# YonkaMayonkaZ/NCF

Hardware: NVIDIA B200
Metric: NeuMF train samples/s (higher is better)
Workload: dtype f32

## Files before the change

### ncf_b200/csrc/tile_umma.cu

```cuda
#include <algorithm>
#include <cstdlib>

#include "common.cuh"
#include "tile_params.cuh"

namespace {

constexpr int kTile = 128;
constexpr uint32_t kHiMask = 0xffffe000u;
constexpr int kProducerWarps = 8;
constexpr int kLoaderWarp = 17;
constexpr int kGemmThreads = 576;
constexpr int kMaxStages = 4;

enum { EPI_RELU_STORE = 0, EPI_PREDICT = 1, EPI_PREDICT_TRAIN = 2, EPI_MASK_STORE = 3, EPI_SCATTER = 4 };

struct GemmArgs {
  int K;
  int N;
  int n_total;
  int passes;
  int layer;
  int gather;
  int stages;
  int ablate;
  const float* a;
  const float* b_img;
  const float* bias;
  float* out;
  const float* mask_src;
};

struct WgradJob {
  int k, mb, nb, cta0, nctas;
  int S;
};
struct WgradArgs {
  int njobs, passes, ablate;
  WgradJob job[12];
};

__device__ __forceinline__ uint32_t smem_u32(const void* p) { return (uint32_t)__cvta_generic_to_shared(p); }

__device__ __forceinline__ void mbar_init(uint64_t* b, uint32_t count) {
  asm volatile("mbarrier.init.shared::cta.b64 [%0], %1;" ::"r"(smem_u32(b)), "r"(count));
}
__device__ __forceinline__ void mbar_arrive(uint64_t* b) {
  asm volatile("mbarrier.arrive.shared::cta.b64 _, [%0];" ::"r"(smem_u32(b)) : "memory");
}
__device__ __forceinline__ void mbar_expect_tx(uint64_t* b, uint32_t bytes) {
  asm volatile("mbarrier.arrive.expect_tx.shared::cta.b64 _, [%0], %1;" ::"r"(smem_u32(b)), "r"(bytes) : "memory");
}
__device__ __forceinline__ void mbar_wait(uint64_t* b, uint32_t parity) {
  const uint32_t addr = smem_u32(b);
  for (uint32_t spin = 0; spin < (1u << 26); ++spin) {
    uint32_t done;
#ifdef NCF_MBAR_POLL
    asm volatile(
        "{\n\t.reg .pred p;\n\tmbarrier.test_wait.parity.shared::cta.b64 p, [%1], %2;\n\tselp.u32 %0, 1, 0, p;\n\t}"
        : "=r"(done) : "r"(addr), "r"(parity) : "memory");
#else
    asm volatile(
        "{\n\t.reg .pred p;\n\tmbarrier.try_wait.parity.shared::cta.b64 p, [%1], %2;\n\tselp.u32 %0, 1, 0, p;\n\t}"
        : "=r"(done) : "r"(addr), "r"(parity) : "memory");
#endif
    if (done) return;
  }
  __trap();
}
__device__ __forceinline__ bool mbar_test_warp(uint64_t* b, uint32_t parity) {
  uint32_t done = 0;
  if ((threadIdx.x & 31) == 0)
    asm volatile(
        "{\n\t.reg .pred p;\n\tmbarrier.test_wait.parity.shared::cta.b64 p, [%1], %2;\n\tselp.u32 %0, 1, 0, p;\n\t}"
        : "=r"(done) : "r"(smem_u32(b)), "r"(parity) : "memory");
  return __shfl_sync(0xffffffffu, done, 0) != 0;
}
__device__ __forceinline__ void mbar_wait_warp(uint64_t* b, uint32_t parity) {
  if ((threadIdx.x & 31) == 0) mbar_wait(b, parity);
  __syncwarp();
}
__device__ __forceinline__ void mbar_arrive_warp(uint64_t* b) {
  __syncwarp();
  if ((threadIdx.x & 31) == 0) mbar_arrive(b);
}
__device__ __forceinline__ void bulk_g2s(void* dst, const void* src, uint32_t bytes, uint64_t* bar) {
  asm volatile("cp.async.bulk.shared::cluster.global.mbarrier::complete_tx::bytes [%0], [%1], %2, [%3];"
               ::"r"(smem_u32(dst)), "l"(src), "r"(bytes), "r"(smem_u32(bar)) : "memory");
}
__device__ __forceinline__ void cp_async16_zfill(void* dst, const void* src, bool valid) {
  asm volatile("cp.async.cg.shared.global [%0], [%1], 16, %2;" ::"r"(smem_u32(dst)), "l"(src), "r"(valid ? 16 : 0) : "memory");
}
__device__ __forceinline__ void fence_async_smem() { asm volatile("fence.proxy.async.shared::cta;" ::: "memory"); }
__device__ __forceinline__ void tc_fence_before() { asm volatile("tcgen05.fence::before_thread_sync;" ::: "memory"); }
__device__ __forceinline__ void tc_fence_after() { asm volatile("tcgen05.fence::after_thread_sync;" ::: "memory"); }
__device__ __forceinline__ void tc_commit(uint64_t* bar) {
  asm volatile("tcgen05.commit.cta_group::1.mbarrier::arrive::one.shared::cluster.b64 [%0];" ::"r"(smem_u32(bar)) : "memory");
}
__device__ __forceinline__ void tc_mma(uint32_t d_tmem, uint64_t da, uint64_t db, uint32_t idesc, uint32_t accumulate) {
  asm volatile(
      "{\n\t.reg .pred p;\n\tsetp.ne.b32 p, %4, 0;\n\t"
      "tcgen05.mma.cta_group::1.kind::tf32 [%0], %1, %2, %3, p;\n\t}"
      ::"r"(d_tmem), "l"(da), "l"(db), "r"(idesc), "r"(accumulate) : "memory");
}
__device__ __forceinline__ void tc_ld32(uint32_t taddr, float (&v)[32]) {
  uint32_t r[32];
  asm volatile(
      "tcgen05.ld.sync.aligned.32x32b.x32.b32 "
      "{%0,%1,%2,%3,%4,%5,%6,%7,%8,%9,%10,%11,%12,%13,%14,%15,"
      "%16,%17,%18,%19,%20,%21,%22,%23,%24,%25,%26,%27,%28,%29,%30,%31}, [%32];"
      : "=r"(r[0]), "=r"(r[1]), "=r"(r[2]), "=r"(r[3]), "=r"(r[4]), "=r"(r[5]), "=r"(r[6]), "=r"(r[7]),
        "=r"(r[8]), "=r"(r[9]), "=r"(r[10]), "=r"(r[11]), "=r"(r[12]), "=r"(r[13]), "=r"(r[14]), "=r"(r[15]),
        "=r"(r[16]), "=r"(r[17]), "=r"(r[18]), "=r"(r[19]), "=r"(r[20]), "=r"(r[21]), "=r"(r[22]), "=r"(r[23]),
        "=r"(r[24]), "=r"(r[25]), "=r"(r[26]), "=r"(r[27]), "=r"(r[28]), "=r"(r[29]), "=r"(r[30]), "=r"(r[31])
      : "r"(taddr));
  asm volatile("tcgen05.wait::ld.sync.aligned;" ::: "memory");
#pragma unroll
  for (int j = 0; j < 32; ++j) v[j] = __uint_as_float(r[j]);
// ... 15 lines not shown
  d |= (uint32_t)a_mn << 15;
  d |= (uint32_t)b_mn << 16;
  d |= (uint32_t)(n >> 3) << 17;
  d |= (uint32_t)(m >> 4) << 24;
  return d;
}

__device__ __forceinline__ void split4(const float4 x, float4& hi, float4& lo) {
  hi.x = __uint_as_float(__float_as_uint(x.x) & kHiMask);
  hi.y = __uint_as_float(__float_as_uint(x.y) & kHiMask);
  hi.z = __uint_as_float(__float_as_uint(x.z) & kHiMask);
  hi.w = __uint_as_float(__float_as_uint(x.w) & kHiMask);
  lo = make_float4(x.x - hi.x, x.y - hi.y, x.z - hi.z, x.w - hi.w);
}

__device__ __forceinline__ float warp_colsum32(float (&v)[32], int lane) {
#pragma unroll
  for (int o = 16; o > 0; o >>= 1) {
    const bool upper = (lane & o) != 0;
#pragma unroll
    for (int i = 0; i < o; ++i) {
      const float send = upper ? v[i] : v[i + o];
      const float keep = upper ? v[i + o] : v[i];
      v[i] = keep + __shfl_xor_sync(0xffffffffu, send, o);
    }
  }
  return v[0];
}

__device__ __forceinline__ void named_bar(int id, int count) {
  asm volatile("bar.sync %0, %1;" ::"r"(id), "r"(count) : "memory");
}

__global__ void umma_weight_images_kernel(const TileParams p) {
  const int k = blockIdx.y >> 1, dir = blockIdx.y & 1;
  const int kin = p.W[k], nout = p.W[k + 1];
  const int rows = dir ? kin : nout, K = dir ? nout : kin;
  const int panels = (K + 31) / 32;
  const float* w = p.w[k];
  float* img = dir ? p.wsplit_b[k] : p.wsplit_f[k];
  const int64_t total = (int64_t)panels * rows * 32;
  for (int64_t idx = blockIdx.x * (int64_t)blockDim.x + threadIdx.x; idx < total;
       idx += (int64_t)gridDim.x * blockDim.x) {
    const int cc = (int)(idx & 31);
    const int r = (int)((idx >> 5) % rows);
    const int pi = (int)((idx >> 5) / rows);
    const int c = pi * 32 + cc;
    float x = 0.f;
    if (c < K) x = dir ? w[(int64_t)c * kin + r] : w[(int64_t)r * kin + c];
    const float hi = __uint_as_float(__float_as_uint(x) & kHiMask);
    const int64_t off = (int64_t)pi * 2 * rows * 32 + (int64_t)r * 32 + ((((cc >> 2) ^ (r & 7)) << 2) | (cc & 3));
    img[off] = hi;
    img[off + (int64_t)rows * 32] = x - hi;
  }
}

#ifdef NCF_UMMA_TRACE
__device__ long long g_trace[3][128];
#define NCF_TRACE(role, slot) do { if (blockIdx.x == 0 && blockIdx.y == 0 && (slot) < 128) g_trace[role][slot] = clock64(); } while (0)
#else
#define NCF_TRACE(role, slot) do { } while (0)
#endif

struct GemmBars {
  uint64_t full[kMaxStages], empty[kMaxStages], acc_full[2], acc_empty[2];
  uint32_t tmem_base;
  float pg[2 * 128 + 4];
// ... 358 lines not shown
          }
        }
      }
      tc_fence_before();
      if (q == 0 && lane == 0) NCF_TRACE(2, 2 * (int)lt + 1);
      mbar_arrive_warp(&bars.acc_empty[a]);
    }
  }
  tc_fence_before();
  __syncthreads();
  if (EPI == EPI_PREDICT_TRAIN)
    for (int i = tid; i <= p.predict_size; i += kGemmThreads) atomicAdd(&p.gt[p.pw_off + i], bars.pg[i]);
  if (warp == kProducerWarps) asm volatile("tcgen05.dealloc.cta_group::1.sync.aligned.b32 %0, %1;" ::"r"(tmem), "r"(tmem_cols));
}

constexpr int kMaxGemms = 2 * NCF_MAX_LAYERS;
constexpr int kRingMax = 6;
constexpr int kBStages = 3;

struct TowerGemm {
  int kind;
  int k, N, K;
  int a_hi, a_lo;
  int d_col;
  int n_total, row0;
  int new_operand;
  const float* img;
};
struct TowerArgs {
  int passes, ng, ablate;
  int ring_col, ring_stages;
  int hcol[NCF_MAX_LAYERS + 1], lcol[NCF_MAX_LAYERS + 1];
  TowerGemm gemm[kMaxGemms];
};

struct TowerBars {
  uint64_t a_full[kRingMax], a_empty[kRingMax], b_full[kBStages], b_empty[kBStages];
  uint64_t acc_ready[2], opnd_ready, tile_done, dl_ready;
  uint64_t panel_ready[8];
  uint32_t tmem_base;
  float pg[2 * 64 + 8];
  float xch[kTile];
};

__device__ __forceinline__ void tc_st32(uint32_t taddr, const float (&v)[32]) {
  asm volatile(
      "tcgen05.st.sync.aligned.32x32b.x32.b32 [%0], {%1,%2,%3,%4,%5,%6,%7,%8,%9,%10,%11,%12,%13,%14,%15,%16,"
      "%17,%18,%19,%20,%21,%22,%23,%24,%25,%26,%27,%28,%29,%30,%31,%32};"
      ::"r"(taddr), "r"(__float_as_uint(v[0])), "r"(__float_as_uint(v[1])), "r"(__float_as_uint(v[2])),
        "r"(__float_as_uint(v[3])), "r"(__float_as_uint(v[4])), "r"(__float_as_uint(v[5])), "r"(__float_as_uint(v[6])),
        "r"(__float_as_uint(v[7])), "r"(__float_as_uint(v[8])), "r"(__float_as_uint(v[9])), "r"(__float_as_uint(v[10])),
        "r"(__float_as_uint(v[11])), "r"(__float_as_uint(v[12])), "r"(__float_as_uint(v[13])), "r"(__float_as_uint(v[14])),
        "r"(__float_as_uint(v[15])), "r"(__float_as_uint(v[16])), "r"(__float_as_uint(v[17])), "r"(__float_as_uint(v[18])),
        "r"(__float_as_uint(v[19])), "r"(__float_as_uint(v[20])), "r"(__float_as_uint(v[21])), "r"(__float_as_uint(v[22])),
        "r"(__float_as_uint(v[23])), "r"(__float_as_uint(v[24])), "r"(__float_as_uint(v[25])), "r"(__float_as_uint(v[26])),
        "r"(__float_as_uint(v[27])), "r"(__float_as_uint(v[28])), "r"(__float_as_uint(v[29])), "r"(__float_as_uint(v[30])),
        "r"(__float_as_uint(v[31])) : "memory");
}
__device__ __forceinline__ void tc_wait_st() { asm volatile("tcgen05.wait::st.sync.aligned;" ::: "memory"); }
__device__ __forceinline__ void tc_mma_ts(uint32_t d_tmem, uint32_t a_tmem, uint64_t db, uint32_t idesc, uint32_t accumulate) {
  asm volatile(
      "{\n\t.reg .pred p;\n\tsetp.ne.b32 p, %4, 0;\n\t"
      "tcgen05.mma.cta_group::1.kind::tf32 [%0], [%1], %2, %3, p;\n\t}"
      ::"r"(d_tmem), "r"(a_tmem), "l"(db), "r"(idesc), "r"(accumulate) : "memory");
}
__device__ __forceinline__ float lo_of(float x) { return x - __uint_as_float(__float_as_uint(x) & kHiMask); }
// ... 36 lines not shown
  extern __shared__ __align__(1024) uint8_t smem_raw[];
  __shared__ TowerBars bars;
  uint8_t* smem = reinterpret_cast<uint8_t*>((reinterpret_cast<uintptr_t>(smem_raw) + 1023) & ~(uintptr_t)1023);
  const int tid = threadIdx.x, warp = tid >> 5, lane = tid & 31;
  const int L = p.L;
  const int64_t ntiles = (p.B + kTile - 1) / kTile;
  const int64_t my_tiles = (blockIdx.x < ntiles) ? (ntiles - blockIdx.x + gridDim.x - 1) / gridDim.x : 0;
  const int P0 = p.W[0] >> 5;
  const uint32_t b_stage = 128u * 256u;
  uint8_t* land = smem + kBStages * b_stage;
  const int NA = g.ring_stages;

  if (tid == 0) {
    const int nm = (g.passes == 3) ? 3 : 1;
    for (int s = 0; s < NA; ++s) { mbar_init(&bars.a_full[s], 4); mbar_init(&bars.a_empty[s], nm); }
    for (int s = 0; s < kBStages; ++s) { mbar_init(&bars.b_full[s], 1); mbar_init(&bars.b_empty[s], nm); }
    mbar_init(&bars.acc_ready[0], nm * kTowerMmaSets);
    mbar_init(&bars.acc_ready[1], nm * kTowerMmaSets);
    mbar_init(&bars.opnd_ready, kTowerEpiWarps);
    for (int c = 0; c < 8; ++c) mbar_init(&bars.panel_ready[c], 4);
    mbar_init(&bars.tile_done, kTowerEpiWarps);
    mbar_init(&bars.dl_ready, kTowerEpiWarps / 2);
    asm volatile("fence.mbarrier_init.release.cluster;" ::: "memory");
  }
  for (int i = tid; i < 2 * 64 + 8; i += kTowerThreads) bars.pg[i] = 0.f;
  if (warp == 8) {
    asm volatile("tcgen05.alloc.cta_group::1.sync.aligned.shared::cta.b32 [%0], 512;" ::"r"(smem_u32(&bars.tmem_base)));
    asm volatile("tcgen05.relinquish_alloc_permit.cta_group::1.sync.aligned;");
  }
  tc_fence_before();
  __syncthreads();
  tc_fence_after();
  const uint32_t tmem = bars.tmem_base;

  if (warp < 8) {
    const int grp = warp >> 2, q = warp & 3;
    const int r = q * 32 + lane;
    const int d = p.d;
    const int own = P0 / 2;
    const uint32_t lane_addr = tmem + ((uint32_t)(q * 32) << 16);
    int s = grp;
    uint32_t ph = 0;
    auto copy_panel = [&](int64_t tl, int pi, int64_t uu, int64_t ii) {
      const bool ok = tl < my_tiles && uu >= 0 && uu < p.U && ii >= 0 && ii < p.I && !(g.ablate & 1);
      const int c0 = pi * 32;
      const float* src = p.eum;
      if (ok) src = (c0 < d) ? p.eum + uu * d + c0 : p.eim + ii * d + (c0 - d);
      uint8_t* dst = land + pi * (kTile * 128) + r * 128;
#pragma unroll
      for (int c = 0; c < 8; ++c) cp_async16_zfill(dst + ((c ^ (r & 7)) << 4), src + c * 4, ok);
      asm volatile("cp.async.commit_group;" ::: "memory");
    };
    auto row_idx = [&](int64_t tl, int64_t& uu, int64_t& ii) {
      uu = -1;
      ii = -1;
      const int64_t row = (blockIdx.x + tl * gridDim.x) * kTile + r;
      if (tl < my_tiles && row < p.B) {
        uu = p.user[p.user_div > 0 ? row / p.user_div : row];
        ii = p.item[row];
      }
    };
    int64_t nu, nit;
    row_idx(0, nu, nit);
    for (int j = 0; j < own; ++j) copy_panel(0, grp + 2 * j, nu, nit);
    const int f = p.f;
    const bool has_gmf = p.type != NCF_MLP;
// ... 338 lines not shown
#pragma unroll
            for (int j = 0; j < 32; ++j) v[j] = (x[j] > 0.f) ? v[j] : 0.f;
            tc_st32(lane_addr + g.lcol[k] + c0, v);
            if (g.passes == 3) {
#pragma unroll
              for (int j = 0; j < 32; ++j) x[j] = lo_of(v[j]);
              tc_st32(lane_addr + g.hcol[k] + c0, x);
            }
            quad8_transpose(v, lane);
            tc_wait_st();
            tc_fence_before();
            mbar_arrive_warp(&bars.panel_ready[c0 >> 5]);
            store_rows_t(v, p.delta[k], N, row - lane, p.B, c0, lane);
          }
        } else {
          for (int c0 = c_begin; c0 < c_end; c0 += 32) {
            tc_ld32(lane_addr + G.d_col + c0, v);
            quad8_transpose(v, lane);
            const int col = G.row0 + c0;
            const bool to_user = col < dmlp;
            const int64_t my_idx = ok ? (to_user ? u : it) : -1;
            float* tab = (to_user ? p.gum + col : p.gim + (col - dmlp)) + 4 * (lane & 7);
#pragma unroll
            for (int i = 0; i < 8; ++i) {
              const int64_t idx = __shfl_sync(0xffffffffu, my_idx, (lane & ~7) + i);
              if (idx >= 0) red_add4(tab + idx * dmlp, make_float4(v[4 * i], v[4 * i + 1], v[4 * i + 2], v[4 * i + 3]));
            }
          }
        }
        if (zero_late) zero_cols(g.gemm[0].d_col, g.gemm[0].N);
        tc_wait_st();
        tc_fence_before();
        if (warp == kTowerEpiWarp0 + 1 && lane == 0) NCF_TRACE(2, 2 * ((int)tl * g.ng + gi) + 1);
        if (gi + 1 == g.ng) mbar_arrive_warp(&bars.tile_done);
      }
    }
  }
  tc_fence_before();
  __syncthreads();
  if (TRAIN)
    for (int i = tid; i <= p.predict_size; i += kTowerThreads) atomicAdd(&p.gt[p.pw_off + i], bars.pg[i]);
  if (warp == 8) asm volatile("tcgen05.dealloc.cta_group::1.sync.aligned.b32 %0, 512;" ::"r"(tmem));
}

constexpr int kWgProducerWarps = 8;
constexpr int kWgProducers = kWgProducerWarps * 32;
constexpr int kWgradThreads = kWgProducers + 96;

constexpr int kWgStages = 2;
struct WgradBars {
  uint64_t full[kWgStages], empty[kWgStages], acc_full;
  uint32_t tmem_base;
  float db[128];
};

__device__ __forceinline__ uint32_t mn_offset(int s, int fo, int S) {
  const int panel = fo >> 5, cc = fo & 31;
  return (uint32_t)(panel * (S * 128) + s * 128 + (((cc >> 3) ^ (s & 3)) << 5) + ((cc & 7) << 2));
}

__global__ void __launch_bounds__(kWgradThreads, 1)
umma_wgrad_kernel(const __grid_constant__ TileParams p, const __grid_constant__ WgradArgs g) {
  extern __shared__ __align__(1024) uint8_t smem_raw[];
  __shared__ WgradBars bars;
  uint8_t* smem = reinterpret_cast<uint8_t*>((reinterpret_cast<uintptr_t>(smem_raw) + 1023) & ~(uintptr_t)1023);
  const int tid = threadIdx.x, warp = tid >> 5, lane = tid & 31;
  int ji = 0;
  while (ji + 1 < g.njobs && (int)blockIdx.x >= g.job[ji + 1].cta0) ++ji;
  const WgradJob job = g.job[ji];
  const int k = job.k, kin = p.W[k], nout = p.W[k + 1];
  const int MB = min(128, nout - job.mb * 128), NB = min(256, kin - job.nb * 256);
  const int local = (int)blockIdx.x - job.cta0;
  const int S = job.S;
  const int64_t nchunks = (p.B + S - 1) / S;
  const uint32_t a_img = (uint32_t)MB * S * 4, b_img = (uint32_t)NB * S * 4;
  const uint32_t stage_bytes = 2 * a_img + 2 * b_img;
  const int64_t my_chunks = (local < nchunks) ? (nchunks - local + job.nctas - 1) / job.nctas : 0;

  if (tid == 0) {
    const int nm = (g.passes == 3) ? 3 : 1;
    for (int s = 0; s < kWgStages; ++s) { mbar_init(&bars.full[s], kWgProducerWarps); mbar_init(&bars.empty[s], nm); }
    mbar_init(&bars.acc_full, nm);
    asm volatile("fence.mbarrier_init.release.cluster;" ::: "memory");
  }
  if (tid < 128) bars.db[tid] = 0.f;
  if (warp == kWgProducerWarps) {
    asm volatile("tcgen05.alloc.cta_group::1.sync.aligned.shared::cta.b32 [%0], 256;" ::"r"(smem_u32(&bars.tmem_base)));
    asm volatile("tcgen05.relinquish_alloc_permit.cta_group::1.sync.aligned;");
  }
  tc_fence_before();
  __syncthreads();
  tc_fence_after();
  const uint32_t tmem = bars.tmem_base;
  if (warp < kWgProducerWarps) {
    float z[32];
#pragma unroll
    for (int j = 0; j < 32; ++j) z[j] = 0.f;
    for (int c0 = (warp >> 2) * 128; c0 < (warp >> 2) * 128 + 128; c0 += 32)
      tc_st32(tmem + ((uint32_t)((warp & 3) * 32) << 16) + c0, z);
    tc_wait_st();
  }
  tc_fence_before();
  __syncthreads();
  tc_fence_after();

  if (warp < kWgProducerWarps) {
    const int t = tid, d = p.d;
    const float* delta = p.delta[k + 1];
    const float* actk = (k > 0) ? p.act[k] : nullptr;
    const int pa = MB >> 2, pb = NB >> 2;
    const int na = S * pa / kWgProducers, nbp = S * pb / kWgProducers;
    const int ca = t % pa, sa0 = t / pa, sas = kWgProducers / pa;
    const int cb = t % pb, sb0 = t / pb, sbs = kWgProducers / pb;
    float4 dbsum = make_float4(0.f, 0.f, 0.f, 0.f);
    const int fo = job.nb * 256 + cb * 4;
    const bool from_user = fo < d;
    const int64_t* idx_src = from_user ? p.user : p.item;
    const float* tab = from_user ? p.eum + fo : p.eim + (fo - d);
    const int64_t idx_lim = from_user ? p.U : p.I;
    int64_t idx_even[8], idx_odd[8];
    auto issue_idx = [&](int64_t ci, int64_t (&idxv)[8]) {
      const int64_t row0 = (local + ci * job.nctas) * S;
#pragma unroll
      for (int i = 0; i < 8; ++i) {
        const int64_t row = row0 + sb0 + i * sbs;
        idxv[i] = (i < nbp && ci < my_chunks && row < p.B) ? idx_src[row] : -1;
      }
    };
    auto issue = [&](int64_t ci, bool blocking) -> bool {
      const int s = (int)(ci % kWgStages);
      const uint32_t par = (uint32_t)((ci / kWgStages) & 1) ^ 1;
      if (blocking) mbar_wait_warp(&bars.empty[s], par);
      else if (!mbar_test_warp(&bars.empty[s], par)) return false;
      if (t == 0) NCF_TRACE(0, 2 * (int)ci);
      uint8_t* st = smem + (size_t)s * stage_bytes;
      const int64_t row0 = (local + ci * job.nctas) * S;
      const bool off = (g.ablate & 64) != 0;
#pragma unroll
      for (int i = 0; i < 4; ++i) {
        if (i < na) {
          const int64_t row = row0 + sa0 + i * sas;
          const bool ok = row < p.B && !off;
          cp_async16_zfill(st + mn_offset(sa0 + i * sas, ca * 4, S),
                           ok ? delta + row * nout + job.mb * 128 + ca * 4 : delta, ok);
        }
      }
#pragma unroll
      for (int i = 0; i < 8; ++i) {
        if (i < nbp) {
          const float* src;
          bool ok;
          if (k == 0) {
            const int64_t ix = (ci & 1) ? idx_odd[i] : idx_even[i];
            ok = ix >= 0 && ix < idx_lim && !off;
            src = ok ? tab + ix * d : tab;
          } else {
            const int64_t row = row0 + sb0 + i * sbs;
            ok = row < p.B && !off;
            src = ok ? actk + row * kin + fo : actk;
          }
          cp_async16_zfill(st + 2 * a_img + mn_offset(sb0 + i * sbs, cb * 4, S), src, ok);
        }
      }
      asm volatile("cp.async.commit_group;" ::: "memory");
      if (k == 0) {
        if (ci & 1) issue_idx(ci + 2, idx_odd);
        else issue_idx(ci + 2, idx_even);
      }
      return true;
    };
    auto consume = [&](int64_t ci, int newer) {
      const int s = (int)(ci % kWgStages);
      uint8_t* st = smem + (size_t)s * stage_bytes;
      if (newer >= 3) asm volatile("cp.async.wait_group 3;" ::: "memory");
      else if (newer == 2) asm volatile("cp.async.wait_group 2;" ::: "memory");
      else if (newer == 1) asm volatile("cp.async.wait_group 1;" ::: "memory");
      else asm volatile("cp.async.wait_group 0;" ::: "memory");
      if (!(g.ablate & 256)) {
#pragma unroll
        for (int i = 0; i < 4; ++i) {
          if (i < na) {
            const uint32_t off = mn_offset(sa0 + i * sas, ca * 4, S);
            const float4 x = *reinterpret_cast<const float4*>(st + off);
            float4 hi, lo;
            split4(x, hi, lo);
            dbsum.x += x.x; dbsum.y += x.y; dbsum.z += x.z; dbsum.w += x.w;
            if (g.ablate & 512) *reinterpret_cast<float4*>(st + off) = x;
            if (g.passes == 3) *reinterpret_cast<float4*>(st + a_img + off) = lo;
          }
        }
#pragma unroll
        for (int i = 0; i < 8; ++i) {
          if (i < nbp && g.passes == 3) {
            const uint32_t off = 2 * a_img + mn_offset(sb0 + i * sbs, cb * 4, S);
            const float4 x = *reinterpret_cast<const float4*>(st + off);
            float4 hi, lo;
            split4(x, hi, lo);
            if (g.ablate & 512) *reinterpret_cast<float4*>(st + off) = x;
            *reinterpret_cast<float4*>(st + b_img + off) = lo;
          }
        }
      }
      fence_async_smem();
      if (t == 0) NCF_TRACE(0, 2 * (int)ci + 1);
      mbar_arrive_warp(&bars.full[s]);
    };
    if (k == 0) {
      issue_idx(0, idx_even);
      issue_idx(1, idx_odd);
    }
    int64_t issued = 0;
    for (int64_t ci = 0; ci < my_chunks; ++ci) {
      if (issued == ci) issue(issued++, true);
      while (issued < my_chunks && issued - ci < kWgStages && issue(issued, false)) ++issued;
      consume(ci, (int)(issued - ci - 1));
    }
    if (job.nb == 0) {
      atomicAdd(&bars.db[ca * 4 + 0], dbsum.x);
      atomicAdd(&bars.db[ca * 4 + 1], dbsum.y);
      atomicAdd(&bars.db[ca * 4 + 2], dbsum.z);
      atomicAdd(&bars.db[ca * 4 + 3], dbsum.w);
    }
    named_bar(1, kWgProducers);
    if (job.nb == 0 && t < MB && my_chunks > 0) atomicAdd(&p.gt[p.b_off[k] + job.mb * 128 + t], bars.db[t]);
    if (my_chunks > 0) {
      mbar_wait_warp(&bars.acc_full, 0);
      tc_fence_after();
      const int q = warp & 3, part = warp >> 2, parts = min(kWgProducerWarps / 4, NB / 32);
      const int m = q * 32 + lane;
      float* dst = p.gt + p.w_off[k] + (int64_t)(job.mb * 128 + m) * kin + job.nb * 256;
      float v[32];
      for (int c0 = part * (NB / parts); c0 < (part + 1) * (NB / parts) && part < parts; c0 += 32) {
        tc_ld32(tmem + ((uint32_t)(q * 32) << 16) + c0, v);
        if (m < MB && !(g.ablate & 32)) {
#pragma unroll
          for (int j = 0; j < 32; j += 4) red_add4(dst + c0 + j, make_float4(v[j], v[j + 1], v[j + 2], v[j + 3]));
        }
      }
    }
  } else if (lane == 0 && (warp == kWgProducerWarps || g.passes == 3)) {
    const int pass = warp - kWgProducerWarps;
    const uint32_t idesc = make_idesc(128, NB, 1, 1);
    for (int64_t ci = 0; ci < my_chunks; ++ci) {
      const int s = (int)(ci % kWgStages);
      mbar_wait(&bars.full[s], (uint32_t)(ci / kWgStages) & 1);
      if (pass == 0) NCF_TRACE(1, 2 * (int)ci);
      tc_fence_after();
      const uint32_t base = smem_u32(smem + (size_t)s * stage_bytes);
      const uint32_t ahi = base, alo = base + a_img, bhi = base + 2 * a_img, blo = bhi + b_img;
      const uint64_t da0 = make_desc(pass == 1 ? alo : ahi, S * 128, 512, 1);
      const uint64_t db0 = make_desc(pass == 2 ? blo : bhi, S * 128, 512, 1);
      for (int ks = 0; ks < ((g.ablate & 128) ? 0 : S / 8); ++ks) tc_mma(tmem, da0 + 64 * ks, db0 + 64 * ks, idesc, 1u);
      tc_commit(&bars.empty[s]);
      if (pass == 0) NCF_TRACE(1, 2 * (int)ci + 1);
    }
    if (my_chunks > 0) tc_commit(&bars.acc_full);
  }
  tc_fence_before();
  __syncthreads();
  if (warp == kWgProducerWarps) asm volatile("tcgen05.dealloc.cta_group::1.sync.aligned.b32 %0, 256;" ::"r"(tmem));
}

constexpr size_t kSmemBudget = 200 * 1024;

static int ablate_knob() {
  static const int v = [] { const char* e = getenv("NCF_UMMA_ABLATE"); return e ? atoi(e) : 0; }();
  return v;
}
static bool timing_knob() {
  static const bool v = getenv("NCF_UMMA_TIMING") != nullptr;
  return v;
}

template <int EPI>
int launch_gemm(const TileParams& p, GemmArgs g, int nblocks, cudaStream_t st) {
  const size_t stage = 2 * (size_t)kTile * 128 + 2 * (size_t)g.N * 128;
  int stages = (int)(kSmemBudget / stage);
  if (stages > kMaxStages) stages = kMaxStages;
  if (stages < 2) {
    ncf::set_error("umma gemm: stage of %zu bytes does not fit twice", stage);
    return NCF_ERR_ARG;
  }
  g.stages = stages;
  g.ablate = ablate_knob();
  const size_t smem = stages * stage + 1024;
  auto kern = umma_gemm_kernel<EPI>;
  NCF_CUDA(cudaFuncSetAttribute(kern, cudaFuncAttributeMaxDynamicSharedMemorySize, (int)smem));
  const int64_t ntiles = (p.B + kTile - 1) / kTile;
  int64_t grid = ncf::num_sms();
  if (grid > ntiles) grid = ntiles;
  kern<<<dim3((unsigned)grid, (unsigned)nblocks), kGemmThreads, smem, st>>>(p, g);
  NCF_LAUNCH_CHECK("umma_gemm_kernel");
#ifdef NCF_UMMA_TRACE
  {
    static int calls = 0;
    const char* want = getenv("NCF_UMMA_TRACE_CALL");
    if (want && atoi(want) == calls) {
      cudaStreamSynchronize(st);
      static long long h[3][128];
      cudaMemcpyFromSymbol(h, g_trace, sizeof(h));
      const long long t0 = h[0][0];
      fprintf(stderr, "[trace] EPI=%d K=%d N=%d stages=%d\n", EPI, g.K, g.N, g.stages);
      for (int i = 0; i < 48; i += 2)
        fprintf(stderr, "[trace] %2d  prod: empty-ok %7lld stored %7lld | mma: full-ok %7lld committed %7lld | epi(tile %d): acc-ok %7lld done %7lld\n",
                i / 2, h[0][i] - t0, h[0][i + 1] - t0, h[1][i] - t0, h[1][i + 1] - t0, i / 2,
                i / 2 < 8 ? h[2][i] - t0 : 0, i / 2 < 8 ? h[2][i + 1] - t0 : 0);
    }
    ++calls;
  }
#endif
  return NCF_OK;
}

int launch_wgrad(const TileParams& p, int passes, cudaStream_t st) {
  WgradArgs g{};
  g.passes = passes;
  g.ablate = ablate_knob();
  double weight[12], total = 0;
  for (int k = 0; k < p.L; ++k) {
    const int mbs = (p.W[k + 1] + 127) / 128, nbs = (p.W[k] + 255) / 256;
    for (int mb = 0; mb < mbs; ++mb)
      for (int nb = 0; nb < nbs; ++nb) {
        if (g.njobs >= 12) {
          ncf::set_error("umma wgrad: too many weight blocks");
          return NCF_ERR_ARG;
        }
        const int MB = std::min(128, p.W[k + 1] - mb * 128), NB = std::min(256, p.W[k] - nb * 256);
        int S = std::min(4096 / MB, 8192 / NB) / 8 * 8;
        S = std::max(8, std::min(S, 256));
        g.job[g.njobs] = WgradJob{k, mb, nb, 0, 0, S};
        weight[g.njobs] = 1.0 / S;
        total += weight[g.njobs];
        ++g.njobs;
      }
  }
  const int sms = ncf::num_sms();
  int cta = 0;
  size_t smem = 0;
  for (int j = 0; j < g.njobs; ++j) {
    const int64_t nchunks = (p.B + g.job[j].S - 1) / g.job[j].S;
    int n = (int)(weight[j] / total * sms);
    if (n < 1) n = 1;
    if (n > nchunks) n = (int)nchunks;
    g.job[j].cta0 = cta;
    g.job[j].nctas = n;
    cta += n;
    const int k = g.job[j].k;
    const int MB = std::min(128, p.W[k + 1] - g.job[j].mb * 128), NB = std::min(256, p.W[k] - g.job[j].nb * 256);
    smem = std::max(smem, (size_t)kWgStages * 2 * (MB + NB) * g.job[j].S * 4);
  }
  smem += 1024;
  NCF_CUDA(cudaFuncSetAttribute(umma_wgrad_kernel, cudaFuncAttributeMaxDynamicSharedMemorySize, (int)smem));
  umma_wgrad_kernel<<<cta, kWgradThreads, smem, st>>>(p, g);
  NCF_LAUNCH_CHECK("umma_wgrad_kernel");
#ifdef NCF_UMMA_TRACE
  if (getenv("NCF_UMMA_TRACE_WGRAD")) {
    cudaStreamSynchronize(st);
    static long long h[3][128];
    cudaMemcpyFromSymbol(h, g_trace, sizeof(h));
    const long long t0 = h[0][0];
    for (int i = 0; i < 48; i += 2)
      fprintf(stderr, "[wtrace] %2d  prod: empty-ok %7lld stored %7lld | mma: full-ok %7lld committed %7lld\n", i / 2,
              h[0][i] - t0, h[0][i + 1] - t0, h[1][i] - t0, h[1][i + 1] - t0);
  }
#endif
  return NCF_OK;
}

struct StepProfile {
  int enabled = 0, n = 0;
  float ms[16];
  const char* name[16];
};
thread_local StepProfile g_profile;

struct StepTimer {
  bool on;
  cudaStream_t st;
  cudaEvent_t ev[32];
  const char* name[32];
  int n = 0;
  static thread_local StepTimer* g_timer;
  StepTimer(cudaStream_t s) : on(g_profile.enabled || timing_knob()), st(s) {
    g_timer = this;
    mark("start");
  }
// ... 37 lines not shown
  g.bias = p.b[k];
  return g;
}

int tower_forward(TileParams& p, int passes, bool train, cudaStream_t st) {
  for (int k = 0; k < p.L; ++k) {
    GemmArgs g = forward_args(p, k, passes);
    int rc;
    if (k + 1 < p.L) {
      g.out = p.act[k + 1];
      rc = launch_gemm<EPI_RELU_STORE>(p, g, g.n_total / g.N, st);
    } else if (train) {
      g.out = p.delta[p.L];
      rc = launch_gemm<EPI_PREDICT_TRAIN>(p, g, 1, st);
    } else {
      rc = launch_gemm<EPI_PREDICT>(p, g, 1, st);
    }
    if (rc != NCF_OK) return rc;
    if (StepTimer::g_timer) StepTimer::g_timer->mark(k == 0 ? "fwd0" : k == 1 ? "fwd1" : "fwd2+");
  }
  return NCF_OK;
}

bool tower_fused_ok(const TileParams& p) {
  const char* off = getenv("NCF_UMMA_FUSED");
  if (off != nullptr && off[0] == '0') return false;
  if (p.W[0] > 256 || p.W[p.L] < 32 || p.f > 64) return false;
  int cols = 0;
  for (int k = 1; k <= p.L; ++k) cols += 2 * p.W[k];
  return cols <= 512 && 2 * p.W[1] + p.W[0] <= 512;
}

template <bool TRAIN>
int launch_tower(const TileParams& p, int passes, cudaStream_t st) {
  TowerArgs g{};
  g.passes = passes;
  g.ablate = ablate_knob();
  int col = 0;
  for (int k = 1; k <= p.L; ++k) {
    g.hcol[k] = col;
    col += p.W[k];
    g.lcol[k] = col;
    col += p.W[k];
  }
  g.ring_col = p.W[1];
  g.ring_stages = std::min(kRingMax, (512 - p.W[1]) / 64);
  for (int k = 0; k < p.L; ++k)
    g.gemm[g.ng++] = TowerGemm{0, k, p.W[k + 1], p.W[k], k == 0 ? -1 : g.hcol[k], k == 0 ? -1 : g.lcol[k],
                               g.hcol[k + 1], p.W[k + 1], 0, k > 0, p.wsplit_f[k]};
  if (TRAIN)
    for (int k = p.L - 1; k >= 0; --k) {
      const bool top = (k + 1 == p.L);
      const int a_hi = top ? g.hcol[p.L] : g.lcol[k + 1], a_lo = top ? g.lcol[p.L] : g.hcol[k + 1];
      for (int n0 = 0; n0 < p.W[k]; n0 += 128) {
        const int N = std::min(128, p.W[k] - n0);
        g.gemm[g.ng++] = TowerGemm{1, k, N, p.W[k + 1], a_hi, a_lo, (k >= 1 ? g.lcol[k] : 2 * p.W[1]) + n0,
                                   p.W[k], n0, n0 == 0, p.wsplit_b[k]};
      }
    }
  const size_t smem = (size_t)kBStages * 128 * 256 + (size_t)(p.W[0] / 32) * kTile * 128 + 1024;
  auto kern = umma_tower_kernel<TRAIN>;
  NCF_CUDA(cudaFuncSetAttribute(kern, cudaFuncAttributeMaxDynamicSharedMemorySize, (int)smem));
  const int64_t ntiles = (p.B + kTile - 1) / kTile;
  int64_t grid = ncf::num_sms();
  if (grid > ntiles) grid = ntiles;
  kern<<<(unsigned)grid, kTowerThreads, smem, st>>>(p, g);
  NCF_LAUNCH_CHECK("umma_tower_kernel");
#ifdef NCF_UMMA_TRACE
  if (getenv("NCF_UMMA_TRACE_TOWER")) {
// ... 22 lines not shown

bool umma_eligible(const TileParams& p) {
  const char* off = getenv("NCF_UMMA_DISABLE");
  if (off != nullptr && off[0] == '1') return false;
  const char* mb = getenv("NCF_UMMA_MIN_B");
  const int64_t min_b = mb ? atoll(mb) : 8192;
  if (p.B < min_b) return false;
  if (p.type == NCF_GMF) return false;
  if (p.f < 32 || p.f > 128 || (p.f & (p.f - 1)) != 0) return false;
  int blocks = 0;
  for (int k = 0; k < p.L; ++k) blocks += ((p.W[k + 1] + 127) / 128) * ((p.W[k] + 255) / 256);
  return blocks <= 12;
}

int64_t umma_image_floats(const TileParams& p) {
  int64_t n = 0;
  for (int k = 0; k < p.L; ++k) n += 2 * 2 * (int64_t)p.W[k] * p.W[k + 1];
  return n;
}

int64_t umma_scratch_floats(const TileParams& p, int64_t B, bool train) {
  int64_t n = 0;
  for (int k = 1; k < p.L; ++k) n += B * p.W[k];
  if (train)
    for (int k = 1; k <= p.L; ++k) n += B * p.W[k];
  return n;
}

constexpr int64_t kForwardSub = 262144;

int64_t umma_forward_workspace_floats(const TileParams& p, int64_t B) {
  return umma_image_floats(p) + umma_scratch_floats(p, std::min<int64_t>(B, kForwardSub), false) + 64;
}
int64_t umma_train_workspace_floats(const TileParams& p, int64_t B) {
  return umma_image_floats(p) + umma_scratch_floats(p, B, true) + 64;
}

static float* carve(TileParams& p, float* ws, int64_t B, bool train, cudaStream_t st, int* rc) {
  for (int k = 0; k < p.L; ++k) {
    const int64_t n = 2 * (int64_t)p.W[k] * p.W[k + 1];
    p.wsplit_f[k] = ws;
    p.wsplit_b[k] = ws + n;
    ws += 2 * n;
  }
  ws = (float*)(((uintptr_t)ws + 255) & ~(uintptr_t)255);
  for (int k = 1; k < p.L; ++k) { p.act[k] = ws; ws += B * p.W[k]; }
  if (train)
    for (int k = 1; k <= p.L; ++k) { p.delta[k] = ws; ws += B * p.W[k]; }
  umma_weight_images_kernel<<<dim3(64, 2 * p.L), 256, 0, st>>>(p);
  *rc = check_cuda(cudaGetLastError(), "umma_weight_images_kernel");
  return ws;
}

int launch_umma_forward(TileParams& p, int passes, float* ws, cudaStream_t st) {
  int rc;
  const int64_t B = p.B;
  if (tower_fused_ok(p)) {
    carve(p, ws, 0, false, st, &rc);
    if (rc != NCF_OK) return rc;
    return launch_tower<false>(p, passes, st);
  }
  int64_t sub = kForwardSub;
  if (p.user_div > 0) sub = std::max<int64_t>(1, sub / p.user_div) * p.user_div;
  carve(p, ws, std::min(B, sub), false, st, &rc);
  if (rc != NCF_OK) return rc;
  const int64_t* user = p.user;
  const int64_t* item = p.item;
  float* logits = p.logits;
  for (int64_t off = 0; off < B; off += sub) {
    p.B = std::min(sub, B - off);
    p.user = (p.user_div > 0) ? user + off / p.user_div : user + off;
    p.item = item + off;
    p.logits = logits + off;
    rc = tower_forward(p, passes, false, st);
    if (rc != NCF_OK) return rc;
  }
  return NCF_OK;
}

int launch_umma_train(TileParams& p, int passes, float* ws, cudaStream_t st) {
  int rc;
  StepTimer timer(st);
  carve(p, ws, p.B, true, st, &rc);
  if (rc != NCF_OK) return rc;
  timer.mark("images");
  if (tower_fused_ok(p)) {
    rc = launch_tower<true>(p, passes, st);
    if (rc != NCF_OK) return rc;
    if ((rc = mark_embedding_grads_done(st)) != NCF_OK) return rc;
    timer.mark("tower");
    rc = launch_wgrad(p, passes, st);
    timer.mark("wgrad");
    return rc;
  }
  rc = tower_forward(p, passes, true, st);
  if (rc != NCF_OK) return rc;
  for (int k = p.L - 1; k >= 0; --k) {
    GemmArgs g{};
    g.K = p.W[k + 1];
    g.n_total = p.W[k];
    g.N = std::min(256, g.n_total);
    g.passes = passes;
    g.layer = k;
    g.a = p.delta[k + 1];
    g.b_img = p.wsplit_b[k];
    if (k > 0) {
      g.out = p.delta[k];
      g.mask_src = p.act[k];
      rc = launch_gemm<EPI_MASK_STORE>(p, g, g.n_total / g.N, st);
    } else {
      rc = launch_gemm<EPI_SCATTER>(p, g, g.n_total / g.N, st);
    }
    if (rc != NCF_OK) return rc;
    timer.mark(k == 2 ? "dgrad2" : k == 1 ? "dgrad1" : k == 0 ? "dgrad0" : "dgrad");
  }
  if ((rc = mark_embedding_grads_done(st)) != NCF_OK) return rc;
  rc = launch_wgrad(p, passes, st);
  timer.mark("wgrad");
  return rc;
}

}

extern "C" int ncf_profile_enable(int32_t on) {
  g_profile.enabled = on;
  g_profile.n = 0;
  return NCF_OK;
}

extern "C" int ncf_profile_read(float* ms, char* names, int32_t cap, int32_t name_len) {
  int n = g_profile.n < cap ? g_profile.n : cap;
  for (int i = 0; i < n; ++i) {
    ms[i] = g_profile.ms[i];
    if (names != nullptr && name_len > 0) snprintf(names + (size_t)i * name_len, name_len, "%s", g_profile.name[i]);
  }
  return n;
}
```

Baseline: 166.2 million.

## Overlap wgrad with fused tower via PDL and per-tile readiness counters

The weight-gradient kernel is launched with programmatic stream serialization so it can start while the fused tower kernel is still running. The tower bumps a per-128-row-tile ready counter after each tile's backward epilogue, and wgrad waits on those counters before using a chunk. Wgrad also changes from a static chunk split to dynamic chunk claiming through a scheduler warp with an atomic per-job counter and an smem ring, and CTAs are interleaved across jobs. The cost is extra spin-waiting, atomics and a possible deadlock if wgrad CTAs take SMs the tower still needs; a NCF_WGRAD_OVERLAP=0 env knob turns the overlap off.

```diff
diff --git a/ncf_b200/csrc/tile_umma.cu b/ncf_b200/csrc/tile_umma.cu
--- a/ncf_b200/csrc/tile_umma.cu
+++ b/ncf_b200/csrc/tile_umma.cu
@@ -32,12 +32,17 @@
 };
 
 struct WgradJob {
-  int k, mb, nb, cta0, nctas;
+  int k, mb, nb;
   int S;
 };
+constexpr int kWgMaxJobs = 12;
+constexpr int kWgMaxCtas = 256;
 struct WgradArgs {
   int njobs, passes, ablate;
-  WgradJob job[12];
+  WgradJob job[kWgMaxJobs];
+  uint32_t* ready;
+  uint32_t* next;
+  uint8_t job_of[kWgMaxCtas];
 };
 
 __device__ __forceinline__ uint32_t smem_u32(const void* p) { return (uint32_t)__cvta_generic_to_shared(p); }
@@ -84,6 +89,15 @@
   __syncwarp();
   if ((threadIdx.x & 31) == 0) mbar_arrive(b);
 }
+__device__ __forceinline__ void wait_count(const uint32_t* c, uint32_t target) {
+  for (uint32_t spin = 0; spin < (1u << 24); ++spin) {
+    uint32_t v;
+    asm volatile("ld.acquire.gpu.global.u32 %0, [%1];" : "=r"(v) : "l"(c) : "memory");
+    if (v >= target) return;
+    __nanosleep(128);
+  }
+  __trap();
+}
 __device__ __forceinline__ void bulk_g2s(void* dst, const void* src, uint32_t bytes, uint64_t* bar) {
   asm volatile("cp.async.bulk.shared::cluster.global.mbarrier::complete_tx::bytes [%0], [%1], %2, [%3];"
                ::"r"(smem_u32(dst)), "l"(src), "r"(bytes), "r"(smem_u32(bar)) : "memory");
@@ -165,7 +179,9 @@
   asm volatile("bar.sync %0, %1;" ::"r"(id), "r"(count) : "memory");
 }
 
-__global__ void umma_weight_images_kernel(const TileParams p) {
+__global__ void umma_weight_images_kernel(const TileParams p, uint32_t* sync, int nsync) {
+  if (blockIdx.y == 0)
+    for (int i = blockIdx.x * blockDim.x + threadIdx.x; i < nsync; i += gridDim.x * blockDim.x) sync[i] = 0;
   const int k = blockIdx.y >> 1, dir = blockIdx.y & 1;
   const int kin = p.W[k], nout = p.W[k + 1];
   const int rows = dir ? kin : nout, K = dir ? nout : kin;
@@ -590,6 +606,7 @@
   int ring_col, ring_stages;
   int hcol[NCF_MAX_LAYERS + 1], lcol[NCF_MAX_LAYERS + 1];
   TowerGemm gemm[kMaxGemms];
+  uint32_t* ready;
 };
 
 struct TowerBars {
@@ -692,6 +709,7 @@
   __syncthreads();
   tc_fence_after();
   const uint32_t tmem = bars.tmem_base;
+  asm volatile("griddepcontrol.launch_dependents;" ::: "memory");
 
   if (warp < 8) {
     const int grp = warp >> 2, q = warp & 3;
@@ -1096,7 +1114,16 @@
         tc_wait_st();
         tc_fence_before();
         if (warp == kTowerEpiWarp0 + 1 && lane == 0) NCF_TRACE(2, 2 * ((int)tl * g.ng + gi) + 1);
-        if (gi + 1 == g.ng) mbar_arrive_warp(&bars.tile_done);
+        if (gi + 1 == g.ng) {
+          mbar_arrive_warp(&bars.tile_done);
+          if (TRAIN) {
+            __syncwarp();
+            if (lane == 0) {
+              __threadfence();
+              atomicAdd(&g.ready[blockIdx.x + tl * gridDim.x], 1u);
+            }
+          }
+        }
       }
     }
   }
@@ -1109,11 +1136,15 @@
 
 constexpr int kWgProducerWarps = 8;
 constexpr int kWgProducers = kWgProducerWarps * 32;
-constexpr int kWgradThreads = kWgProducers + 96;
+constexpr int kWgSchedWarp = kWgProducerWarps + 3;
+constexpr int kWgradThreads = kWgProducers + 128;
+constexpr int kWgRing = 4;
 
 constexpr int kWgStages = 2;
 struct WgradBars {
   uint64_t full[kWgStages], empty[kWgStages], acc_full;
+  uint64_t cid_full[kWgRing], cid_empty[kWgRing];
+  int32_t cid[kWgRing];
   uint32_t tmem_base;
   float db[128];
 };
@@ -1129,22 +1160,20 @@
   __shared__ WgradBars bars;
   uint8_t* smem = reinterpret_cast<uint8_t*>((reinterpret_cast<uintptr_t>(smem_raw) + 1023) & ~(uintptr_t)1023);
   const int tid = threadIdx.x, warp = tid >> 5, lane = tid & 31;
-  int ji = 0;
-  while (ji + 1 < g.njobs && (int)blockIdx.x >= g.job[ji + 1].cta0) ++ji;
+  const int ji = g.job_of[blockIdx.x];
   const WgradJob job = g.job[ji];
   const int k = job.k, kin = p.W[k], nout = p.W[k + 1];
   const int MB = min(128, nout - job.mb * 128), NB = min(256, kin - job.nb * 256);
-  const int local = (int)blockIdx.x - job.cta0;
   const int S = job.S;
   const int64_t nchunks = (p.B + S - 1) / S;
   const uint32_t a_img = (uint32_t)MB * S * 4, b_img = (uint32_t)NB * S * 4;
   const uint32_t stage_bytes = 2 * a_img + 2 * b_img;
-  const int64_t my_chunks = (local < nchunks) ? (nchunks - local + job.nctas - 1) / job.nctas : 0;
 
   if (tid == 0) {
     const int nm = (g.passes == 3) ? 3 : 1;
     for (int s = 0; s < kWgStages; ++s) { mbar_init(&bars.full[s], kWgProducerWarps); mbar_init(&bars.empty[s], nm); }
     mbar_init(&bars.acc_full, nm);
+    for (int r = 0; r < kWgRing; ++r) { mbar_init(&bars.cid_full[r], 1); mbar_init(&bars.cid_empty[r], kWgProducerWarps + nm); }
     asm volatile("fence.mbarrier_init.release.cluster;" ::: "memory");
   }
   if (tid < 128) bars.db[tid] = 0.f;
@@ -1182,23 +1211,39 @@
     const int64_t* idx_src = from_user ? p.user : p.item;
     const float* tab = from_user ? p.eum + fo : p.eim + (fo - d);
     const int64_t idx_lim = from_user ? p.U : p.I;
+    int64_t n_end = INT64_MAX;
+    auto chunk_of = [&](int64_t n, bool blocking) -> int64_t {
+      if (n > n_end) return -1;
+      const int r = (int)(n % kWgRing);
+      const uint32_t par = (uint32_t)(n / kWgRing) & 1;
+      if (blocking) mbar_wait_warp(&bars.cid_full[r], par);
+      else if (!mbar_test_warp(&bars.cid_full[r], par)) return -2;
+      __syncwarp();
+      const int64_t c = bars.cid[r];
+      if (c < 0) n_end = n;
+      return c;
+    };
     int64_t idx_even[8], idx_odd[8];
     auto issue_idx = [&](int64_t ci, int64_t (&idxv)[8]) {
-      const int64_t row0 = (local + ci * job.nctas) * S;
+      const int64_t c = chunk_of(ci, true);
+      const int64_t row0 = c * S;
 #pragma unroll
       for (int i = 0; i < 8; ++i) {
         const int64_t row = row0 + sb0 + i * sbs;
-        idxv[i] = (i < nbp && ci < my_chunks && row < p.B) ? idx_src[row] : -1;
+        idxv[i] = (i < nbp && c >= 0 && row < p.B) ? idx_src[row] : -1;
       }
     };
     auto issue = [&](int64_t ci, bool blocking) -> bool {
       const int s = (int)(ci % kWgStages);
       const uint32_t par = (uint32_t)((ci / kWgStages) & 1) ^ 1;
+      if (!blocking && !mbar_test_warp(&bars.empty[s], par)) return false;
+      const int64_t c = chunk_of(ci, blocking);
+      if (c < 0) return false;
       if (blocking) mbar_wait_warp(&bars.empty[s], par);
-      else if (!mbar_test_warp(&bars.empty[s], par)) return false;
       if (t == 0) NCF_TRACE(0, 2 * (int)ci);
       uint8_t* st = smem + (size_t)s * stage_bytes;
-      const int64_t row0 = (local + ci * job.nctas) * S;
+      const int64_t row0 = c * S;
+      mbar_arrive_warp(&bars.cid_empty[ci % kWgRing]);
       const bool off = (g.ablate & 64) != 0;
 #pragma unroll
       for (int i = 0; i < 4; ++i) {
@@ -1228,6 +1273,7 @@
       }
       asm volatile("cp.async.commit_group;" ::: "memory");
       if (k == 0) {
+        chunk_of(ci + 1, true);
         if (ci & 1) issue_idx(ci + 2, idx_odd);
         else issue_idx(ci + 2, idx_even);
       }
@@ -1273,11 +1319,14 @@
       issue_idx(0, idx_even);
       issue_idx(1, idx_odd);
     }
-    int64_t issued = 0;
-    for (int64_t ci = 0; ci < my_chunks; ++ci) {
-      if (issued == ci) issue(issued++, true);
-      while (issued < my_chunks && issued - ci < kWgStages && issue(issued, false)) ++issued;
-      consume(ci, (int)(issued - ci - 1));
+    int64_t issued = 0, my_chunks = 0;
+    for (;; ++my_chunks) {
+      if (issued == my_chunks) {
+        if (!issue(issued, true)) break;
+        ++issued;
+      }
+      while (issued - my_chunks < kWgStages && issue(issued, false)) ++issued;
+      consume(my_chunks, (int)(issued - my_chunks - 1));
     }
     if (job.nb == 0) {
       atomicAdd(&bars.db[ca * 4 + 0], dbsum.x);
@@ -1302,10 +1351,32 @@
         }
       }
     }
+  } else if (warp == kWgSchedWarp) {
+    if (lane == 0) {
+      int64_t c = atomicAdd(&g.next[ji], 1u);
+      for (int64_t n = 0;; ++n) {
+        const bool more = c < nchunks;
+        const int64_t cn = more ? atomicAdd(&g.next[ji], 1u) : c;
+        if (more && g.ready != nullptr)
+          for (int64_t tl = c * S / kTile; tl <= (min((c + 1) * S, p.B) - 1) / kTile; ++tl) wait_count(&g.ready[tl], kTowerEpiWarps);
+        const int r = (int)(n % kWgRing);
+        mbar_wait(&bars.cid_empty[r], ((uint32_t)(n / kWgRing) & 1) ^ 1);
+        bars.cid[r] = more ? (int32_t)c : -1;
+        mbar_arrive(&bars.cid_full[r]);
+        if (!more) break;
+        c = cn;
+      }
+    }
   } else if (lane == 0 && (warp == kWgProducerWarps || g.passes == 3)) {
     const int pass = warp - kWgProducerWarps;
     const uint32_t idesc = make_idesc(128, NB, 1, 1);
-    for (int64_t ci = 0; ci < my_chunks; ++ci) {
+    int64_t ci = 0;
+    for (;; ++ci) {
+      const int r = (int)(ci % kWgRing);
+      mbar_wait(&bars.cid_full[r], (uint32_t)(ci / kWgRing) & 1);
+      const bool more = bars.cid[r] >= 0;
+      mbar_arrive(&bars.cid_empty[r]);
+      if (!more) break;
       const int s = (int)(ci % kWgStages);
       mbar_wait(&bars.full[s], (uint32_t)(ci / kWgStages) & 1);
       if (pass == 0) NCF_TRACE(1, 2 * (int)ci);
@@ -1318,11 +1389,12 @@
       tc_commit(&bars.empty[s]);
       if (pass == 0) NCF_TRACE(1, 2 * (int)ci + 1);
     }
-    if (my_chunks > 0) tc_commit(&bars.acc_full);
+    if (ci > 0) tc_commit(&bars.acc_full);
   }
   tc_fence_before();
   __syncthreads();
   if (warp == kWgProducerWarps) asm volatile("tcgen05.dealloc.cta_group::1.sync.aligned.b32 %0, 256;" ::"r"(tmem));
+  asm volatile("griddepcontrol.wait;" ::: "memory");
 }
 
 constexpr size_t kSmemBudget = 200 * 1024;
@@ -1333,6 +1405,10 @@
 }
 static bool timing_knob() {
   static const bool v = getenv("NCF_UMMA_TIMING") != nullptr;
+  return v;
+}
+static bool wgrad_overlap_knob() {
+  static const bool v = [] { const char* e = getenv("NCF_WGRAD_OVERLAP"); return !(e && e[0] == '0'); }();
   return v;
 }
 
@@ -1376,46 +1452,79 @@
   return NCF_OK;
 }
 
-int launch_wgrad(const TileParams& p, int passes, cudaStream_t st) {
+int launch_wgrad(const TileParams& p, int passes, uint32_t* ready, uint32_t* next, cudaStream_t st) {
   WgradArgs g{};
   g.passes = passes;
   g.ablate = ablate_knob();
+  g.ready = ready;
+  g.next = next;
   double weight[12], total = 0;
   for (int k = 0; k < p.L; ++k) {
     const int mbs = (p.W[k + 1] + 127) / 128, nbs = (p.W[k] + 255) / 256;
     for (int mb = 0; mb < mbs; ++mb)
       for (int nb = 0; nb < nbs; ++nb) {
-        if (g.njobs >= 12) {
+        if (g.njobs >= kWgMaxJobs) {
           ncf::set_error("umma wgrad: too many weight blocks");
           return NCF_ERR_ARG;
         }
         const int MB = std::min(128, p.W[k + 1] - mb * 128), NB = std::min(256, p.W[k] - nb * 256);
         int S = std::min(4096 / MB, 8192 / NB) / 8 * 8;
         S = std::max(8, std::min(S, 256));
-        g.job[g.njobs] = WgradJob{k, mb, nb, 0, 0, S};
+        g.job[g.njobs] = WgradJob{k, mb, nb, S};
         weight[g.njobs] = 1.0 / S;
         total += weight[g.njobs];
         ++g.njobs;
       }
   }
   const int sms = ncf::num_sms();
-  int cta = 0;
+  int n[kWgMaxJobs], cta = 0;
+  int64_t nchunks[kWgMaxJobs];
+  for (int j = 0; j < g.njobs; ++j) {
+    nchunks[j] = (p.B + g.job[j].S - 1) / g.job[j].S;
+    n[j] = (int)std::min<int64_t>(std::max(1, (int)(weight[j] / total * sms)), nchunks[j]);
+    cta += n[j];
+  }
+  for (; cta < sms; ++cta) {
+    int best = -1;
+    for (int j = 0; j < g.njobs; ++j)
+      if (n[j] < nchunks[j] && (best < 0 || weight[j] / n[j] > weight[best] / n[best])) best = j;
+    if (best < 0) break;
+    ++n[best];
+  }
+  if (cta > kWgMaxCtas) {
+    ncf::set_error("umma wgrad: %d CTAs exceed the job map", cta);
+    return NCF_ERR_ARG;
+  }
+  int given[kWgMaxJobs] = {};
+  for (int b = 0; b < cta; ++b) {
+    int best = -1;
+    double best_def = 0;
+    for (int j = 0; j < g.njobs; ++j) {
+      const double def = (double)(b + 1) * n[j] / cta - given[j];
+      if (given[j] < n[j] && (best < 0 || def > best_def)) { best = j; best_def = def; }
+    }
+    g.job_of[b] = (uint8_t)best;
+    ++given[best];
+  }
   size_t smem = 0;
   for (int j = 0; j < g.njobs; ++j) {
-    const int64_t nchunks = (p.B + g.job[j].S - 1) / g.job[j].S;
-    int n = (int)(weight[j] / total * sms);
-    if (n < 1) n = 1;
-    if (n > nchunks) n = (int)nchunks;
-    g.job[j].cta0 = cta;
-    g.job[j].nctas = n;
-    cta += n;
     const int k = g.job[j].k;
     const int MB = std::min(128, p.W[k + 1] - g.job[j].mb * 128), NB = std::min(256, p.W[k] - g.job[j].nb * 256);
     smem = std::max(smem, (size_t)kWgStages * 2 * (MB + NB) * g.job[j].S * 4);
   }
   smem += 1024;
   NCF_CUDA(cudaFuncSetAttribute(umma_wgrad_kernel, cudaFuncAttributeMaxDynamicSharedMemorySize, (int)smem));
-  umma_wgrad_kernel<<<cta, kWgradThreads, smem, st>>>(p, g);
+  cudaLaunchConfig_t cfg{};
+  cfg.gridDim = dim3((unsigned)cta);
+  cfg.blockDim = dim3(kWgradThreads);
+  cfg.dynamicSmemBytes = smem;
+  cfg.stream = st;
+  cudaLaunchAttribute attr[1];
+  attr[0].id = cudaLaunchAttributeProgrammaticStreamSerialization;
+  attr[0].val.programmaticStreamSerializationAllowed = 1;
+  cfg.attrs = attr;
+  cfg.numAttrs = (ready != nullptr && wgrad_overlap_knob()) ? 1 : 0;
+  NCF_CUDA(cudaLaunchKernelEx(&cfg, umma_wgrad_kernel, p, g));
   NCF_LAUNCH_CHECK("umma_wgrad_kernel");
 #ifdef NCF_UMMA_TRACE
   if (getenv("NCF_UMMA_TRACE_WGRAD")) {
@@ -1519,9 +1628,10 @@
 }
 
 template <bool TRAIN>
-int launch_tower(const TileParams& p, int passes, cudaStream_t st) {
+int launch_tower(const TileParams& p, int passes, uint32_t* ready, cudaStream_t st) {
   TowerArgs g{};
   g.passes = passes;
+  g.ready = ready;
   g.ablate = ablate_knob();
   int col = 0;
   for (int k = 1; k <= p.L; ++k) {
@@ -1610,11 +1720,13 @@
 int64_t umma_forward_workspace_floats(const TileParams& p, int64_t B) {
   return umma_image_floats(p) + umma_scratch_floats(p, std::min<int64_t>(B, kForwardSub), false) + 64;
 }
+static int64_t sync_count(int64_t B) { return (B + kTile - 1) / kTile + kWgMaxJobs; }
+
 int64_t umma_train_workspace_floats(const TileParams& p, int64_t B) {
-  return umma_image_floats(p) + umma_scratch_floats(p, B, true) + 64;
-}
-
-static float* carve(TileParams& p, float* ws, int64_t B, bool train, cudaStream_t st, int* rc) {
+  return umma_image_floats(p) + umma_scratch_floats(p, B, true) + sync_count(B) + 64;
+}
+
+static uint32_t* carve(TileParams& p, float* ws, int64_t B, bool train, cudaStream_t st, int* rc) {
   for (int k = 0; k < p.L; ++k) {
     const int64_t n = 2 * (int64_t)p.W[k] * p.W[k + 1];
     p.wsplit_f[k] = ws;
@@ -1625,9 +1737,10 @@
   for (int k = 1; k < p.L; ++k) { p.act[k] = ws; ws += B * p.W[k]; }
   if (train)
     for (int k = 1; k <= p.L; ++k) { p.delta[k] = ws; ws += B * p.W[k]; }
-  umma_weight_images_kernel<<<dim3(64, 2 * p.L), 256, 0, st>>>(p);
+  uint32_t* sync = train ? reinterpret_cast<uint32_t*>(ws) : nullptr;
+  umma_weight_images_kernel<<<dim3(64, 2 * p.L), 256, 0, st>>>(p, sync, train ? (int)sync_count(B) : 0);
   *rc = check_cuda(cudaGetLastError(), "umma_weight_images_kernel");
-  return ws;
+  return sync;
 }
 
 int launch_umma_forward(TileParams& p, int passes, float* ws, cudaStream_t st) {
@@ -1636,7 +1749,7 @@
   if (tower_fused_ok(p)) {
     carve(p, ws, 0, false, st, &rc);
     if (rc != NCF_OK) return rc;
-    return launch_tower<false>(p, passes, st);
+    return launch_tower<false>(p, passes, nullptr, st);
   }
   int64_t sub = kForwardSub;
   if (p.user_div > 0) sub = std::max<int64_t>(1, sub / p.user_div) * p.user_div;
@@ -1659,15 +1772,17 @@
 int launch_umma_train(TileParams& p, int passes, float* ws, cudaStream_t st) {
   int rc;
   StepTimer timer(st);
-  carve(p, ws, p.B, true, st, &rc);
+  uint32_t* sync = carve(p, ws, p.B, true, st, &rc);
   if (rc != NCF_OK) return rc;
+  uint32_t* ready = sync;
+  uint32_t* next = sync + sync_count(p.B) - kWgMaxJobs;
   timer.mark("images");
   if (tower_fused_ok(p)) {
-    rc = launch_tower<true>(p, passes, st);
+    rc = launch_tower<true>(p, passes, ready, st);
     if (rc != NCF_OK) return rc;
     if ((rc = mark_embedding_grads_done(st)) != NCF_OK) return rc;
     timer.mark("tower");
-    rc = launch_wgrad(p, passes, st);
+    rc = launch_wgrad(p, passes, ready, next, st);
     timer.mark("wgrad");
     return rc;
   }
@@ -1693,7 +1808,7 @@
     timer.mark(k == 2 ? "dgrad2" : k == 1 ? "dgrad1" : k == 0 ? "dgrad0" : "dgrad");
   }
   if ((rc = mark_embedding_grads_done(st)) != NCF_OK) return rc;
-  rc = launch_wgrad(p, passes, st);
+  rc = launch_wgrad(p, passes, nullptr, next, st);
   timer.mark("wgrad");
   return rc;
 }
```

Result: faster. 168.4 million (median of 6 runs) (+1.3%).
